# dark-Stallion/alac

Measured on AMD Instinct MI355X. Metric: encode Msamples/s (bit-exact) 44.1kHz/16-bit stereo, 1/2/4/8 GPU, higher is better.
Workload: dtype int32 (int16 PCM, int16 coefficients)

## Files before the change

alac_amd/csrc/alac_golomb.hpp:

```cpp
#pragma once

#include "alac_dev.hpp"

namespace alacdev {

__device__ __forceinline__ void gol_table_init(uint32_t *recip, int tid)
{
    if (tid < 17) {
        const uint64_t m = (1ull << tid) - 1;
        recip[tid] = tid >= 2 ? (uint32_t)(((1ull << 32) + m - 1) / m) : 0u;
    }
}

struct GolF {
    uint32_t mb, zmode, inrun, nz1, bits;
    uint64_t acc;
    uint32_t nacc, wleft;
    uint32_t *wp;
    uint32_t *wlim;
    uint32_t q0, q1, q2, q3, qn;
};

__device__ __forceinline__ void golf_reset(GolF &g)
{
    g.mb = kMB0;
    g.zmode = 0;
    g.inrun = 0;
    g.nz1 = 1;
    g.bits = 0;
    g.acc = 0;
    g.nacc = 0;
    g.wleft = 0;
    g.wp = nullptr;
    g.wlim = nullptr;
    g.q0 = g.q1 = g.q2 = g.q3 = g.qn = 0;
}

template <bool WRITE, bool LAZY = false>
__device__ __forceinline__ void golf_put(GolF &g, uint32_t value, uint32_t nbits)
{
    if constexpr (!WRITE) g.bits += nbits;
    if constexpr (WRITE) {
        g.acc = (g.acc << nbits) | (uint64_t)value;
        g.nacc += nbits;
        const uint32_t word = (uint32_t)((g.acc << ((64u - g.nacc) & 63u)) >> 32);
        if constexpr (LAZY) {
            const bool full = (g.nacc >> 5) != 0;
            g.q0 = full ? g.q1 : g.q0;
            g.q1 = full ? g.q2 : g.q1;
            g.q2 = full ? g.q3 : g.q2;
            g.q3 = full ? word : g.q3;
            g.qn += full ? 1u : 0u;
            if (g.qn == 4) {
                *(uint4 *)g.wp = make_uint4(g.q0, g.q1, g.q2, g.q3);
                const uint32_t adv = g.wleft >= 4 ? 4u : 0u;
                g.wleft -= adv;
                g.wp += adv;
                g.qn = 0;
            }
        } else {
            *g.wp = word;
            g.wp += g.nacc >> 5;
        }
        g.nacc &= 31u;
    }
}

__device__ __forceinline__ void golf_open(GolF &g, uint32_t *slot, uint32_t wcap)
{
    g.wp = slot;
    g.wlim = slot + (wcap - 34);
    g.wleft = wcap - 1;
}

template <bool LAZY = false>
__device__ __forceinline__ uint32_t golf_written_bits(const GolF &g, const uint32_t *slot)
{
    return 32u * ((uint32_t)(g.wp - slot) + (LAZY ? g.qn : 0u)) + g.nacc;
}

template <bool WRITE, bool LAZY = false>
__device__ __forceinline__ void golf_flush(GolF &g)
{
    if constexpr (WRITE) {
        if constexpr (LAZY) {
            if (g.qn == 3) g.wp[0] = g.q1;
            if (g.qn >= 2) g.wp[g.qn - 2] = g.q2;
            if (g.qn >= 1) g.wp[g.qn - 1] = g.q3;
            if (g.nacc > 0) g.wp[g.qn] = (uint32_t)((g.acc << (64u - g.nacc)) >> 32);
        } else {
            if (g.nacc > 0) *g.wp = (uint32_t)((g.acc << (64u - g.nacc)) >> 32);
        }
    }
}

template <bool WRITE, bool LAZY = false>
__device__ __forceinline__ void golf_close_run(GolF &g, const uint32_t *recip)
{
    const uint32_t k = (uint32_t)(lead(g.mb) - 24 + (int32_t)((g.mb + 16u) >> 6));
    const uint32_t mz = (1u << k) - 1;
    const uint32_t nz = g.nz1 - 1;
    const uint32_t div = __umulhi(nz, recip[k]);
    uint32_t numBits, value;
    if (div >= kMaxPrefix) {
        numBits = kMaxPrefix + kMaxRunBits;
        value = (((1u << kMaxPrefix) - 1) << kMaxRunBits) + nz;
    } else {
        const uint32_t mod = nz - div * mz;
        const uint32_t de = (mod == 0);
        numBits = div + k + 1 - de;
        value = (((1u << div) - 1) << (numBits - div)) + mod + 1 - de;
    }
    golf_put<WRITE, LAZY>(g, value, numBits);
    g.mb = 0;
    g.inrun = 0;
}

template <bool WRITE, bool CHECKED, bool ZZ = false, bool LAZY = false>
__device__ __forceinline__ void golf_sym(GolF &g, int32_t del, bool valid, uint32_t bitSize, const uint32_t *recip)
{
    const uint32_t t2 = ZZ ? (uint32_t)del : (((uint32_t)del << 1) ^ (uint32_t)(del >> 31));
    uint32_t nzf;
    asm("v_min_u32 %0, 1, %1" : "=v"(nzf) : "v"(t2));
    const uint32_t inr = CHECKED ? (valid ? g.inrun : 0u) : g.inrun;
    const uint32_t sw = inr & (nzf ^ 1u);
    g.nz1 += sw;
    const uint32_t cl = inr & (nzf | (g.nz1 >> 16));
    if (cl) {
        const uint32_t capf = sw;
        golf_close_run<WRITE, LAZY>(g, recip);
        if (capf) g.zmode = 0;
    }
    asm volatile("" : "+v"(g.mb));
    const bool live = CHECKED ? (valid && !sw) : !sw;
    if (CHECKED ? live : true) {
        const uint32_t k = min(22u - (uint32_t)__builtin_clz(g.mb + (3u << kQBShift)), kKB0);
        const uint32_t m = (1u << k) - 1;
        const uint32_t n = t2 - g.zmode;
        const bool esc = n >= m * 9;
        const uint32_t d1 = (n + (n >> k) + 1u) >> k;
        const uint32_t div = (n + d1 + 1u) >> k;
        const uint32_t mod = n - __umul24(div, m);
        const uint32_t ne = min(mod, 1u);
        const uint32_t kd = k + ne;
        uint32_t numBits = div + kd;
        uint32_t value = (((1u << div) - 1) << kd) + mod + ne;
        if (esc) {
            numBits = kMaxPrefix + bitSize;
            value = (((1u << kMaxPrefix) - 1) << bitSize) | (n & ((1u << bitSize) - 1));
        }
        if (!live) {
            numBits = 0;
            value = 0;
        }
        golf_put<WRITE, LAZY>(g, value, numBits);
        uint32_t mb = __umul24(t2, 40u) + g.mb - (times5(g.mb) >> (kQBShift - 3));
        mb = n > kMeanClamp ? kMeanClamp : mb;
        const bool enter = mb < (1u << (kQBShift - 2));
        g.mb = live ? mb : g.mb;
        g.zmode = live ? (enter ? 1u : 0u) : g.zmode;
        g.inrun = live ? (enter ? 1u : 0u) : g.inrun;
        g.nz1 = (live && enter) ? 1u : g.nz1;
    }
}

template <bool WRITE, bool LAZY = false>
__device__ __forceinline__ void golf_finish(GolF &g, bool active, const uint32_t *recip)
{
    const bool close = active && g.inrun && g.nz1 > 1;
    if (__any(close)) {
        if (close) golf_close_run<WRITE, LAZY>(g, recip);
    }
    g.inrun = 0;
}

__device__ __forceinline__ uint32_t wave_min_u32(uint32_t v)
{
#pragma unroll
    for (int d = 32; d > 0; d >>= 1) v = min(v, (uint32_t)__shfl_xor((int)v, d));
    return (uint32_t)__builtin_amdgcn_readfirstlane((int)v);
}

struct NoWait {
    __device__ __forceinline__ void operator()(uint32_t) const {}
};

struct RowSrc {
    const int32_t *p0, *p1;
    uint64_t s0, s1;
    uint32_t split;
    uint32_t col;
};

__device__ __forceinline__ RowSrc one_plane(const int32_t *plane, uint64_t stride, uint32_t col)
{
    RowSrc r;
    r.p0 = r.p1 = plane;
    r.s0 = r.s1 = stride;
    r.split = 0xffffffffu;
    r.col = col;
    return r;
}

template <bool WRITE, bool ZZ = false, class Need = NoWait, bool LAZY = false>
__device__ __forceinline__ void golf_stream(GolF &g, uint32_t n, uint32_t nMaxWave, uint32_t bitSize,
                                            const uint32_t *recip, const RowSrc &R, Need &&need = Need(),
                                            bool idleFast = true, bool finish = true)
{
    constexpr int B = 16;
    int32_t bufA[B], bufB[B], bufC[B];
    auto load = [&](int32_t (&buf)[B], uint32_t jb) {
        if (jb < nMaxWave) {
            need(min(jb + B, nMaxWave));
            if (jb + B <= R.split || jb >= R.split) {
                const bool first = jb + B <= R.split;
                const uint64_t st = first ? R.s0 : R.s1;
                const char *base = (const char *)((first ? R.p0 : R.p1) + (uint64_t)jb * st);
                const uint32_t rowBytes = (uint32_t)st * 4u;
                uint32_t off = R.col * 4u;
#pragma unroll
                for (int s = 0; s < B; s++) {
                    buf[s] = *(const int32_t *)(base + off);
                    off += rowBytes;
                }
            } else {
#pragma unroll
                for (int s = 0; s < B; s++) {
                    const uint32_t j = jb + s;
                    buf[s] = (j < R.split ? R.p0 + (uint64_t)j * R.s0 : R.p1 + (uint64_t)j * R.s1)[R.col];
                }
            }
        }
    };
    const uint32_t nMinWave = wave_min_u32(n ? n : (idleFast ? 0xffffffffu : 0u));
    auto guard = [&]() {
        if constexpr (WRITE && !LAZY) g.wp = g.wp < g.wlim ? g.wp : g.wlim;
    };
    auto codeFast = [&](const int32_t (&buf)[B]) {
        guard();
#pragma unroll
        for (int s = 0; s < B; s++) golf_sym<WRITE, false, ZZ, LAZY>(g, buf[s], true, bitSize, recip);
    };
    auto codeChecked = [&](const int32_t (&buf)[B], uint32_t jb) {
        if (jb >= nMaxWave) return;
        guard();
#pragma unroll
        for (int s = 0; s < B; s++) golf_sym<WRITE, true, ZZ, LAZY>(g, buf[s], jb + s < n, bitSize, recip);
    };
    const uint32_t fastEnd = (min(nMinWave, nMaxWave) / (3 * B)) * (3 * B);
    load(bufA, 0);
    load(bufB, B);
    uint32_t jb = 0;
    for (; jb < fastEnd; jb += 3 * B) {
        load(bufC, jb + 2 * B);
        codeFast(bufA);
        load(bufA, jb + 3 * B);
        codeFast(bufB);
        load(bufB, jb + 4 * B);
        codeFast(bufC);
    }
    for (; jb < nMaxWave; jb += 3 * B) {
        load(bufC, jb + 2 * B);
        codeChecked(bufA, jb);
        load(bufA, jb + 3 * B);
        codeChecked(bufB, jb + B);
        load(bufB, jb + 4 * B);
        codeChecked(bufC, jb + 2 * B);
    }
    const uint32_t openRun = g.inrun;
    golf_finish<WRITE, LAZY>(g, n > 0 && finish, recip);
    if (!finish) g.inrun = openRun;
}

template <bool WRITE, class Fetch, class Need = NoWait>
__device__ __forceinline__ void golf_stream_fn(GolF &g, uint32_t n, uint32_t nMaxWave, uint32_t bitSize,
                                            const uint32_t *recip, Fetch &&fetch, Need &&need = Need(), bool idleFast = true,
                                            bool finish = true)
{
    constexpr int B = 16;
    int32_t bufA[B], bufB[B], bufC[B];
    auto load = [&](int32_t (&buf)[B], uint32_t jb) {
        if (jb < nMaxWave) {
            need(min(jb + B, nMaxWave));
#pragma unroll
            for (int s = 0; s < B; s++) buf[s] = fetch(jb + s);
        }
    };
    const uint32_t nMinWave = wave_min_u32(n ? n : (idleFast ? 0xffffffffu : 0u));
    auto code = [&](const int32_t (&buf)[B], uint32_t jb) {
        if (jb >= nMaxWave) return;
        if (jb + B <= nMinWave) {
#pragma unroll
            for (int s = 0; s < B; s++) golf_sym<WRITE, false>(g, buf[s], true, bitSize, recip);
        } else {
#pragma unroll
            for (int s = 0; s < B; s++) golf_sym<WRITE, true>(g, buf[s], jb + s < n, bitSize, recip);
        }
    };
    load(bufA, 0);
    load(bufB, B);
    for (uint32_t jb = 0; jb < nMaxWave; jb += 3 * B) {
        load(bufC, jb + 2 * B);
        code(bufA, jb);
        load(bufA, jb + 3 * B);
        code(bufB, jb + B);
        load(bufB, jb + 4 * B);
        code(bufC, jb + 2 * B);
    }
    const uint32_t openRun = g.inrun;
    golf_finish<WRITE>(g, n > 0 && finish, recip);
    if (!finish) g.inrun = openRun;
}

}
```

alac_amd/csrc/alac_lpc.hip:

```cpp
#include "alac_dev.hpp"
#include "alac_golomb.hpp"
#include "alac_kernels.hpp"
#include "alac_taps.hpp"

namespace alacdev {

using namespace taps;

namespace {

constexpr int kLags = kLpcMaxOrder + 1;
constexpr int kCands = 6;
constexpr int kWavesPerChan = 3;
constexpr int kChanThreads = 64 * kWavesPerChan;
__constant__ int kOrders[kCands] = {4, 8, 12, 16, 24, 30};

struct Cand {
    int32_t den;
    int16_t coefs[32];
};

template <bool WRITE>
__device__ uint32_t lpc_pass(const int32_t *X, uint32_t N, const Cand &cd, int na, int k, uint32_t chanBits,
                             const uint32_t *recip, uint32_t *slot, uint32_t wcap)
{
    const uint32_t chanshift = 32 - chanBits;
    int32_t a = k < na ? (int32_t)cd.coefs[k] : 0;
    int32_t x = 0;
    GolF g;
    golf_reset(g);
    if constexpr (WRITE) golf_open(g, slot, wcap);
    for (uint32_t j = 0; j < N; j++) {
        const int32_t cur = X[j];
        int32_t del;
        if (j > (uint32_t)na) {
            del = taps_step(cur, x, a, na, k, chanshift, (uint32_t)cd.den);
        } else {
            const int32_t prev = __shfl(x, 0, 32);
            del = j == 0 ? cur : sext(cur - prev, chanshift);
        }
        x = taps_slide(x, cur, k);
        if constexpr (WRITE)
            if ((j & 15) == 0) g.wp = g.wp < g.wlim ? g.wp : g.wlim;
        golf_sym<WRITE, false>(g, del, true, chanBits, recip);
    }
    golf_finish<WRITE>(g, N > 0, recip);
    if constexpr (WRITE) {
        golf_flush<WRITE>(g);
        return golf_written_bits(g, slot);
    }
    return g.bits;
}

__device__ void lpc_levinson(const double *r, uint32_t N, Cand *cand)
{
    for (int c = 0; c < kCands; c++) cand[c].den = 0;
    if (!(r[0] > 0.0)) return;
    double a[kLags] = {0}, t[kLags];
    double err = r[0];
    int next = 0;
    for (int m = 1; m <= kLpcMaxOrder && next < kCands; m++) {
        double acc = r[m];
        for (int i = 1; i < m; i++) acc -= a[i] * r[m - i];
        const double km = acc / err;
        if (!(fabs(km) < 1.0)) return;
        for (int i = 1; i < m; i++) t[i] = a[i] - km * a[m - i];
        for (int i = 1; i < m; i++) a[i] = t[i];
        a[m] = km;
        err *= 1.0 - km * km;
        if (!(err > 0.0)) return;
        if (m != kOrders[next]) continue;
        Cand &cd = cand[next++];
        if (2u * (uint32_t)m >= N) return;
        double amax = 0;
        for (int i = 1; i <= m; i++) amax = fmax(amax, fabs(a[i]));
        int den = 15;
        while (den >= 5 && rint(amax * (double)(1 << den)) > 32767.0) den--;
        if (den < 5) continue;
        for (int i = 1; i <= m; i++) cd.coefs[i - 1] = (int16_t)rint(a[i] * (double)(1 << den));
        cd.den = den;
    }
}

}

template <int DEPTH, int CH>
__global__ __launch_bounds__(kChanThreads * CH) void k_lpc(LpcArgs A)
{
    extern __shared__ int32_t planes[];
    __shared__ uint32_t recip[17];
    __shared__ double part[CH][kWavesPerChan][kLags];
    __shared__ Cand cand[CH][kCands];
    __shared__ uint32_t bits[CH][kCands];
    __shared__ int32_t win[CH];
    constexpr uint32_t SHB = bytes_shifted(DEPTH);
    constexpr uint32_t chanBits = DEPTH - 8 * SHB + (CH == 2 ? 1 : 0);
    const uint32_t p = blockIdx.x, tid = threadIdx.x;
    const uint32_t c = tid / kChanThreads, tc = tid - c * kChanThreads, wave = tc >> 6, lane = tc & 63;
    const int k = (int)(lane & 31), h = (int)(wave * 2 + (lane >> 5));
    PacketRec *rec = A.recs + p;
    if (tid < CH) A.lpc[(uint64_t)p * 2 + tid].num = 0;
    const uint32_t N = rec->numSamples, mixRes = rec->mixRes;
    if (rec->escape || N == 0 || N > A.frameSize) return;
    gol_table_init(recip, (int)tid);
    int32_t *X = planes + c * A.frameSize;
    const uint8_t *pk = A.pcm + (uint64_t)p * A.frameSize * CH * bytes_per_sample(DEPTH);
    for (uint32_t j = tc; j < N; j += kChanThreads) {
        if constexpr (CH == 2) {
            int32_t l, r;
            load_lr<DEPTH>(pk, j, l, r);
            X[j] = mix_sample((int32_t)mixRes, (int)c, l, r);
        } else {
            X[j] = load_sample<DEPTH>(pk, j) >> (8 * (int)SHB);
        }
    }
    __syncthreads();

    double acc[kLags];
#pragma unroll
    for (int L = 0; L < kLags; L++) acc[L] = 0.0;
    for (uint32_t j = tc; j < N; j += kChanThreads) {
        const double xj = (double)X[j];
#pragma unroll
        for (int L = 0; L < kLags; L++)
            if (j >= (uint32_t)L) acc[L] = fma(xj, (double)X[j - L], acc[L]);
    }
#pragma unroll
    for (int L = 0; L < kLags; L++) {
        double v = acc[L];
#pragma unroll
        for (int d = 32; d >= 1; d >>= 1) v += __shfl_xor(v, d);
        if (lane == 0) part[c][wave][L] = v;
    }
    __syncthreads();
    if (tc == 0) {
        double r[kLags];
        for (int L = 0; L < kLags; L++) r[L] = (part[c][0][L] + part[c][1][L]) + part[c][2][L];
        lpc_levinson(r, N, cand[c]);
    }
    __syncthreads();

    const Cand &cd = cand[c][h];
    const int na = kOrders[h];
    const bool live = cd.den != 0;
    if (live) {
        const uint32_t b = lpc_pass<false>(X, N, cd, na, k, chanBits, recip, nullptr, 0);
        if (k == 0) bits[c][h] = b;
    }
    __syncthreads();
    if (tc == 0) {
        uint32_t best = 16u * rec->c[c].num + rec->c[c].bits;
        int w = -1;
        for (int q = 0; q < kCands; q++) {
            if (!cand[c][q].den) continue;
            const uint32_t cost = 16u * (uint32_t)kOrders[q] + bits[c][q];
            if (cost < best) best = cost, w = q;
        }
        win[c] = w;
    }
    __syncthreads();
    if (win[c] == h) {
        uint32_t *slot = A.bitWords + ((uint64_t)p * 2 + c) * A.wcap;
        const uint32_t b = lpc_pass<true>(X, N, cd, na, k, chanBits, recip, slot, A.wcap);
        if (k == 0) {
            rec->c[c].bits = b;
            rec->c[c].num = (uint16_t)na;
            LpcChan &o = A.lpc[(uint64_t)p * 2 + c];
            o.den = (uint16_t)cd.den;
            for (int i = 0; i < na; i++) o.coefs[i] = cd.coefs[i];
            o.num = (uint16_t)na;
        }
    }
    __syncthreads();
    if (tid == 0 && (win[0] >= 0 || win[CH - 1] >= 0)) {
        const uint32_t partial = (N != A.frameSize);
        uint32_t body = 12 + 4 + (partial ? 32 : 0) + 16 + N * (SHB * 8) * CH;
        for (uint32_t q = 0; q < (uint32_t)CH; q++) body += 16 + 16 * rec->c[q].num + rec->c[q].bits;
        rec->totalBits = 7 + body + 3;
        A.packetBytes[p] = (7 + body + 3 + 7) / 8;
    }
}

template <int DEPTH>
static void launch_lpc_depth(uint32_t channels, const LpcArgs &a, uint32_t numPackets, hipStream_t st)
{
    const size_t lds = (size_t)channels * a.frameSize * 4;
    if (channels == 2)
        hipLaunchKernelGGL((k_lpc<DEPTH, 2>), dim3(numPackets), dim3(2 * kChanThreads), lds, st, a);
    else
        hipLaunchKernelGGL((k_lpc<DEPTH, 1>), dim3(numPackets), dim3(kChanThreads), lds, st, a);
}

hipError_t launch_lpc(uint32_t depth, uint32_t channels, const LpcArgs &a, uint32_t numPackets, hipStream_t st)
{
    if (numPackets == 0) return hipSuccess;
    switch (depth) {
    case 16: launch_lpc_depth<16>(channels, a, numPackets, st); break;
    case 20: launch_lpc_depth<20>(channels, a, numPackets, st); break;
    case 24: launch_lpc_depth<24>(channels, a, numPackets, st); break;
    case 32: launch_lpc_depth<32>(channels, a, numPackets, st); break;
    default: return hipErrorInvalidValue;
    }
    return hipGetLastError();
}

}
```

Before: 28550.

## Replace 64-bit bit accumulator with 32-bit alignbit writer and merged run state

The Golomb-Rice bit writer drops its 64-bit accumulator and write-pointer advance. It now keeps a 32-bit carry word and a running bit count, uses alignbit to form output words and indexes the slot by bits>>5. The zmode, inrun and nz1 run-tracking fields are folded into one nz1 counter whose high half flags a run close, and the coding maths uses bfm and add3 intrinsics. The aim is to cut VALU instructions and registers per symbol in the serial entropy-coding loop, at the cost of subtle bit-exactness risks in the reordered run/clamp logic.

New measurement: 28340 (median of 6 runs). No clear change (-0.8%).

```diff
diff --git a/alac_amd/csrc/alac_golomb.hpp b/alac_amd/csrc/alac_golomb.hpp
--- a/alac_amd/csrc/alac_golomb.hpp
+++ b/alac_amd/csrc/alac_golomb.hpp
@@ -13,27 +13,47 @@
 }
 
 struct GolF {
-    uint32_t mb, zmode, inrun, nz1, bits;
-    uint64_t acc;
-    uint32_t nacc, wleft;
+    uint32_t mb;
+    uint32_t nz1;
+    uint32_t bits;
+    uint32_t cur;
+    uint32_t blim;
+    uint32_t wleft;
     uint32_t *wp;
-    uint32_t *wlim;
     uint32_t q0, q1, q2, q3, qn;
 };
 
 __device__ __forceinline__ void golf_reset(GolF &g)
 {
     g.mb = kMB0;
-    g.zmode = 0;
-    g.inrun = 0;
-    g.nz1 = 1;
+    g.nz1 = 0;
     g.bits = 0;
-    g.acc = 0;
-    g.nacc = 0;
+    g.cur = 0;
+    g.blim = 0;
     g.wleft = 0;
     g.wp = nullptr;
-    g.wlim = nullptr;
     g.q0 = g.q1 = g.q2 = g.q3 = g.qn = 0;
+}
+
+__device__ __forceinline__ uint32_t bfm(uint32_t w, uint32_t s)
+{
+    uint32_t r;
+    asm("v_bfm_b32 %0, %1, %2" : "=v"(r) : "v"(w), "v"(s));
+    return r;
+}
+
+__device__ __forceinline__ uint32_t min1(uint32_t x)
+{
+    uint32_t r;
+    asm("v_min_u32 %0, 1, %1" : "=v"(r) : "v"(x));
+    return r;
+}
+
+__device__ __forceinline__ uint32_t add3(uint32_t a, uint32_t b, uint32_t c)
+{
+    uint32_t r;
+    asm("v_add3_u32 %0, %1, %2, %3" : "=v"(r) : "v"(a), "v"(b), "v"(c));
+    return r;
 }
 
 template <bool WRITE, bool LAZY = false>
@@ -41,11 +61,12 @@
 {
     if constexpr (!WRITE) g.bits += nbits;
     if constexpr (WRITE) {
-        g.acc = (g.acc << nbits) | (uint64_t)value;
-        g.nacc += nbits;
-        const uint32_t word = (uint32_t)((g.acc << ((64u - g.nacc) & 63u)) >> 32);
+        const uint32_t sh = 0u - nbits;
+        const uint32_t va = value << (sh & 31u);
+        const uint32_t word = __builtin_amdgcn_alignbit(g.cur, va, g.bits);
+        g.cur = __builtin_amdgcn_alignbit(g.cur, va, sh);
         if constexpr (LAZY) {
-            const bool full = (g.nacc >> 5) != 0;
+            const bool full = (((g.bits & 31u) + nbits) >> 5) != 0;
             g.q0 = full ? g.q1 : g.q0;
             g.q1 = full ? g.q2 : g.q1;
             g.q2 = full ? g.q3 : g.q2;
@@ -59,37 +80,48 @@
                 g.qn = 0;
             }
         } else {
-            *g.wp = word;
-            g.wp += g.nacc >> 5;
-        }
-        g.nacc &= 31u;
+            uint32_t w;
+            asm("v_lshrrev_b32 %0, 5, %1" : "=v"(w) : "v"(g.bits));
+            g.wp[w] = word;
+        }
+        g.bits += nbits;
     }
 }
 
 __device__ __forceinline__ void golf_open(GolF &g, uint32_t *slot, uint32_t wcap)
 {
     g.wp = slot;
-    g.wlim = slot + (wcap - 34);
+    g.bits = 0;
+    g.cur = 0;
+    g.blim = 32u * (wcap - 34);
     g.wleft = wcap - 1;
 }
 
+template <bool WRITE, bool LAZY = false>
+__device__ __forceinline__ void golf_guard(GolF &g)
+{
+    if constexpr (WRITE && !LAZY) g.bits = min(g.bits, g.blim);
+}
+
 template <bool LAZY = false>
-__device__ __forceinline__ uint32_t golf_written_bits(const GolF &g, const uint32_t *slot)
-{
-    return 32u * ((uint32_t)(g.wp - slot) + (LAZY ? g.qn : 0u)) + g.nacc;
+__device__ __forceinline__ uint32_t golf_written_bits(const GolF &g, const uint32_t *)
+{
+    return g.bits;
 }
 
 template <bool WRITE, bool LAZY = false>
 __device__ __forceinline__ void golf_flush(GolF &g)
 {
     if constexpr (WRITE) {
+        const uint32_t nacc = g.bits & 31u;
+        const uint32_t last = nacc ? g.cur << (32u - nacc) : 0u;
         if constexpr (LAZY) {
             if (g.qn == 3) g.wp[0] = g.q1;
             if (g.qn >= 2) g.wp[g.qn - 2] = g.q2;
             if (g.qn >= 1) g.wp[g.qn - 1] = g.q3;
-            if (g.nacc > 0) g.wp[g.qn] = (uint32_t)((g.acc << (64u - g.nacc)) >> 32);
+            if (nacc > 0) g.wp[g.qn] = last;
         } else {
-            if (g.nacc > 0) *g.wp = (uint32_t)((g.acc << (64u - g.nacc)) >> 32);
+            if (nacc > 0) g.wp[g.bits >> 5] = last;
         }
     }
 }
@@ -99,7 +131,7 @@
 {
     const uint32_t k = (uint32_t)(lead(g.mb) - 24 + (int32_t)((g.mb + 16u) >> 6));
     const uint32_t mz = (1u << k) - 1;
-    const uint32_t nz = g.nz1 - 1;
+    const uint32_t nz = (g.nz1 > 0x10000u ? g.nz1 - 0x10000u : g.nz1) - 1;
     const uint32_t div = __umulhi(nz, recip[k]);
     uint32_t numBits, value;
     if (div >= kMaxPrefix) {
@@ -113,65 +145,57 @@
     }
     golf_put<WRITE, LAZY>(g, value, numBits);
     g.mb = 0;
-    g.inrun = 0;
+    g.nz1 = 0;
 }
 
 template <bool WRITE, bool CHECKED, bool ZZ = false, bool LAZY = false>
 __device__ __forceinline__ void golf_sym(GolF &g, int32_t del, bool valid, uint32_t bitSize, const uint32_t *recip)
 {
     const uint32_t t2 = ZZ ? (uint32_t)del : (((uint32_t)del << 1) ^ (uint32_t)(del >> 31));
-    uint32_t nzf;
-    asm("v_min_u32 %0, 1, %1" : "=v"(nzf) : "v"(t2));
-    const uint32_t inr = CHECKED ? (valid ? g.inrun : 0u) : g.inrun;
-    const uint32_t sw = inr & (nzf ^ 1u);
-    g.nz1 += sw;
-    const uint32_t cl = inr & (nzf | (g.nz1 >> 16));
-    if (cl) {
-        const uint32_t capf = sw;
-        golf_close_run<WRITE, LAZY>(g, recip);
-        if (capf) g.zmode = 0;
-    }
+    const uint32_t nzf = min1(t2);
+    const uint32_t inr = CHECKED ? (valid ? min1(g.nz1) : 0u) : min1(g.nz1);
+    g.nz1 += inr << (nzf << 4);
+    const bool cl = g.nz1 > 0xffffu;
+    if (cl) golf_close_run<WRITE, LAZY>(g, recip);
     asm volatile("" : "+v"(g.mb));
-    const bool live = CHECKED ? (valid && !sw) : !sw;
+    const bool live = CHECKED ? (valid && inr <= nzf) : inr <= nzf;
     if (CHECKED ? live : true) {
         const uint32_t k = min(22u - (uint32_t)__builtin_clz(g.mb + (3u << kQBShift)), kKB0);
-        const uint32_t m = (1u << k) - 1;
-        const uint32_t n = t2 - g.zmode;
-        const bool esc = n >= m * 9;
-        const uint32_t d1 = (n + (n >> k) + 1u) >> k;
-        const uint32_t div = (n + d1 + 1u) >> k;
+        const uint32_t m = bfm(k, 0u);
+        const uint32_t n = t2 - inr;
+        const bool esc = n >= __umul24(m, 9u);
+        const uint32_t d1 = add3(n, n >> k, 1u) >> k;
+        const uint32_t div = add3(n, d1, 1u) >> k;
         const uint32_t mod = n - __umul24(div, m);
-        const uint32_t ne = min(mod, 1u);
+        const uint32_t ne = min1(mod);
         const uint32_t kd = k + ne;
         uint32_t numBits = div + kd;
-        uint32_t value = (((1u << div) - 1) << kd) + mod + ne;
+        uint32_t value = add3(bfm(div, kd), mod, ne);
         if (esc) {
             numBits = kMaxPrefix + bitSize;
-            value = (((1u << kMaxPrefix) - 1) << bitSize) | (n & ((1u << bitSize) - 1));
+            value = n | (~0u << bitSize);
         }
         if (!live) {
             numBits = 0;
-            value = 0;
+            value = g.cur;
         }
         golf_put<WRITE, LAZY>(g, value, numBits);
         uint32_t mb = __umul24(t2, 40u) + g.mb - (times5(g.mb) >> (kQBShift - 3));
+        const bool enter = mb < (1u << (kQBShift - 2));
         mb = n > kMeanClamp ? kMeanClamp : mb;
-        const bool enter = mb < (1u << (kQBShift - 2));
         g.mb = live ? mb : g.mb;
-        g.zmode = live ? (enter ? 1u : 0u) : g.zmode;
-        g.inrun = live ? (enter ? 1u : 0u) : g.inrun;
-        g.nz1 = (live && enter) ? 1u : g.nz1;
+        g.nz1 = live ? (enter ? 1u : 0u) : g.nz1;
     }
 }
 
 template <bool WRITE, bool LAZY = false>
 __device__ __forceinline__ void golf_finish(GolF &g, bool active, const uint32_t *recip)
 {
-    const bool close = active && g.inrun && g.nz1 > 1;
+    const bool close = active && g.nz1 > 1;
     if (__any(close)) {
         if (close) golf_close_run<WRITE, LAZY>(g, recip);
     }
-    g.inrun = 0;
+    g.nz1 = 0;
 }
 
 __device__ __forceinline__ uint32_t wave_min_u32(uint32_t v)
@@ -233,9 +257,7 @@
         }
     };
     const uint32_t nMinWave = wave_min_u32(n ? n : (idleFast ? 0xffffffffu : 0u));
-    auto guard = [&]() {
-        if constexpr (WRITE && !LAZY) g.wp = g.wp < g.wlim ? g.wp : g.wlim;
-    };
+    auto guard = [&]() { golf_guard<WRITE, LAZY>(g); };
     auto codeFast = [&](const int32_t (&buf)[B]) {
         guard();
 #pragma unroll
@@ -267,9 +289,9 @@
         load(bufB, jb + 4 * B);
         codeChecked(bufC, jb + 2 * B);
     }
-    const uint32_t openRun = g.inrun;
+    const uint32_t openRun = g.nz1;
     golf_finish<WRITE, LAZY>(g, n > 0 && finish, recip);
-    if (!finish) g.inrun = openRun;
+    if (!finish) g.nz1 = openRun;
 }
 
 template <bool WRITE, class Fetch, class Need = NoWait>
@@ -307,9 +329,9 @@
         load(bufB, jb + 4 * B);
         code(bufC, jb + 2 * B);
     }
-    const uint32_t openRun = g.inrun;
+    const uint32_t openRun = g.nz1;
     golf_finish<WRITE>(g, n > 0 && finish, recip);
-    if (!finish) g.inrun = openRun;
-}
-
-}
+    if (!finish) g.nz1 = openRun;
+}
+
+}
diff --git a/alac_amd/csrc/alac_lpc.hip b/alac_amd/csrc/alac_lpc.hip
--- a/alac_amd/csrc/alac_lpc.hip
+++ b/alac_amd/csrc/alac_lpc.hip
@@ -40,8 +40,7 @@
             del = j == 0 ? cur : sext(cur - prev, chanshift);
         }
         x = taps_slide(x, cur, k);
-        if constexpr (WRITE)
-            if ((j & 15) == 0) g.wp = g.wp < g.wlim ? g.wp : g.wlim;
+        if ((j & 15) == 0) golf_guard<WRITE>(g);
         golf_sym<WRITE, false>(g, del, true, chanBits, recip);
     }
     golf_finish<WRITE>(g, N > 0, recip);
```
